# NERSC/swin_v2_weather

Measured on AMD Instinct MI355X. Metric: ERA5 samples/sec (73x721x1440) swin_73var depth12, higher is better.
Workload: dtype bf16

## Files before the change

### swin_v2_weather_amd/csrc/attn_bwd_stream.hip

```cpp
#include <stdlib.h>

#include "attn_common.h"

namespace {

typedef __attribute__((address_space(3))) unsigned lds_u32;

#ifdef SWV2_ATTNS_ARRIVE
__device__ unsigned long long attns_arr[17 * 8];
#endif

#ifdef SWV2_ATTNS_STAMPS
__device__ unsigned long long attns_stamps[512 * 8];
__device__ unsigned long long attns_win[64 * 128];
__device__ unsigned long long attns_clock[512 * 2];
#define SSTAMP_DECL unsigned long long st_prev = 0, st_acc[8] = {0, 0, 0, 0, 0, 0, 0, 0};
#define SSTAMP_START() do { asm volatile("s_memtime %0\n\ts_waitcnt lgkmcnt(0)" : "=s"(st_prev) : : "memory"); } while (0)
#define SSTAMP(k) do { unsigned long long t_; asm volatile("s_memtime %0\n\ts_waitcnt lgkmcnt(0)" : "=s"(t_) : : "memory"); \
                       st_acc[k] += t_ - st_prev; st_prev = t_; } while (0)
#else
#define SSTAMP_DECL
#define SSTAMP_START() do {} while (0)
#define SSTAMP(k) do {} while (0)
#endif
// ... 29 lines not shown
    const int lane = tid & 63;
    const int tw = __builtin_amdgcn_readfirstlane(tid >> 6);
    const int hd = blockIdx.y;
    const bool helper = tw >= PW;
    const int hw = tw - PW;

    const float tau = logit_scale[hd];
    const float sigma = __expf(fminf(tau, SWV2_LN100));
    const float sc2 = sigma * SWV2_LOG2E;
    const float inv_sc2 = 1.f / sc2;
    const int Lc = LFIX > 0 ? LFIX : L;

    if (tid < 8) ((unsigned*)(lds + OFF_CNT))[tid] = 0u;
    const unsigned lds_base = (unsigned)(uintptr_t)(lds_u32*)lds;
    const unsigned cnt_addr = lds_base + OFF_CNT;

    struct Stg { uint4 q, dO, o; float lse, rn; };
    Stg s0, s1;
    const bool two = helper && hw == HW - 1;
    auto issue = [&](int bw, int nbuf, int hidx) {
        const size_t item = (size_t)__builtin_amdgcn_readfirstlane(bw) * h + hd;
        const char* const qb = (const char*)(qkvh + item * 3 * SLAB);
        unsigned kofs = SLAB * 2, vofs = 2 * SLAB * 2;
        asm volatile("" : "+s"(kofs), "+s"(vofs));
        const char* const kb_ = qb + kofs;
        const char* const vb_ = qb + vofs;
        const char* const dob = (const char*)(doh + item * SLAB);
        const char* const ob = (const char*)(oh + item * SLAB);
        auto one = [&](Stg& st, const int craw, const unsigned lds_k) {
            const int c = min(craw, CH - 1);
            unsigned o16 = (unsigned)c * 16u, ol = (unsigned)(c / CPR) * 4u, orn = (unsigned)c * 4u;
            asm volatile("" : "+v"(o16), "+v"(ol), "+v"(orn));
            if (craw < CH) {
                asm volatile("s_mov_b32 m0, %2\n\ts_nop 0\n\tglobal_load_lds_dwordx4 %0, %1" : : "v"(o16), "s"(kb_), "s"(lds_k) : "memory");
                asm volatile("s_mov_b32 m0, %2\n\ts_nop 0\n\tglobal_load_lds_dwordx4 %0, %1" : : "v"(o16), "s"(vb_), "s"(lds_k + SLAB * 2) : "memory");
            }
            st.q = *(const uint4*)(qb + o16);
            st.dO = *(const uint4*)(dob + o16);
            st.o = *(const uint4*)(ob + o16);
            st.lse = *(const float*)((const char*)(lse + item * Lp) + ol);
            st.rn = *(const float*)((const char*)(rnorm + item * 2 * Lp) + orn);
        };
        const unsigned lds_k0 = lds_base + (unsigned)(nbuf * BUFB + B_K);
        one(s0, hidx, lds_k0 + (unsigned)hw * 1024u);
        if (two) one(s1, HT + (hidx & 63), lds_k0 + (unsigned)HT * 16u);
    };
    auto commit = [&](int buf, int hidx) {
        unsigned char* const B = lds + buf * BUFB;
        auto one = [&](const Stg& st, const int craw) {
            const int c = min(craw, CH - 1);
            const int row = c / CPR, half = c % CPR;
            float dl = 0.f;
            {
                const uint32_t a[4] = {st.dO.x, st.dO.y, st.dO.z, st.dO.w}, b[4] = {st.o.x, st.o.y, st.o.z, st.o.w};
#pragma unroll
                for (int e = 0; e < 4; ++e) {
                    dl = fmaf(__uint_as_float(a[e] << 16), __uint_as_float(b[e] << 16), dl);
                    dl = fmaf(__uint_as_float(a[e] & 0xffff0000u), __uint_as_float(b[e] & 0xffff0000u), dl);
                }
            }
            dl = group_allsum<CPR>(dl);
            uint4 aq = make_uint4(0, 0, 0, 0), ad = make_uint4(0, 0, 0, 0);
            if (half == 0) {
                const bool q_ok = row < L;
                const float lq = q_ok ? st.lse * inv_sc2 : 1.0e30f;
                uint16_t l0 = f2bf(lq);
                const float r1 = lq - bf2f(l0);
                uint16_t l1 = f2bf(r1), l2 = f2bf(r1 - bf2f(l1));
                if (!q_ok) l1 = l2 = 0;
                const uint16_t d0 = f2bf(dl);
                const float e1 = dl - bf2f(d0);
                const uint16_t d1 = f2bf(e1), d2 = f2bf(e1 - bf2f(d1));
                const uint32_t one_ = 0x3f80u, rqf = (row >= mask_thr) ? 0x3f80u : 0u;
                aq = make_uint4(l0 | ((uint32_t)l1 << 16), l2 | (one_ << 16), rqf | ((one_ - rqf) << 16), 0);
                ad = make_uint4(d0 | ((uint32_t)d1 << 16), d2, 0, 0);
            }
            if (craw < CH) {
                *(uint4*)((uint16_t*)(B + B_Q) + row * QP + half * 8) = st.q;
                *(uint4*)((uint16_t*)(B + B_DO) + row * QP + half * 8) = st.dO;
                *(uint4*)((uint16_t*)(B + B_Q) + row * QP + QSTAT + half * 8) = aq;
                *(uint4*)((uint16_t*)(B + B_DO) + row * QP + QSTAT + half * 8) = ad;
                ((float*)(B + B_RN))[c] = st.rn;
            }
        };
        one(s0, hidx);
        if (two) one(s1, HT + (hidx & 63));
    };

    int bw = blockIdx.x;
    if (bw >= Bw) return;
    if (helper) {
        issue(bw, 0, hw * 64 + lane);
        commit(0, hw * 64 + lane);
    }
    __syncthreads();

    float dsig = 0.f;
    SSTAMP_DECL
    SSTAMP_START();
#ifdef SWV2_ATTNS_STAMPS
    const unsigned long long ck0 = __builtin_amdgcn_s_memtime(), rt0 = __builtin_amdgcn_s_memrealtime();
#endif
    for (int it = 0; bw < Bw; bw += gridDim.x, ++it) {
        const int buf = it & 1;
        const size_t slab0 = ((size_t)bw * h + hd) * 3 * SLAB;
        const int bw_next = bw + gridDim.x;
        const unsigned char* const B = lds + buf * BUFB;
        const uint16_t* const Qa = (const uint16_t*)(B + B_Q);
        const uint16_t* const Da = (const uint16_t*)(B + B_DO);
        const uint16_t* const Ks = (const uint16_t*)(B + B_K);
        const uint16_t* const Vs = (const uint16_t*)(B + B_V);
        const float* const RN = (const float*)(B + B_RN);
        const unsigned target = (unsigned)(PW * (it + 1));

        int ln = lane;
        asm volatile("" : "+v"(ln));
        const int fr = ln & 15, g = ln >> 4;
        auto phase2 = [&](const int qt0, auto nq_c, auto sleep_c) {
            constexpr int NQ = decltype(nq_c)::value;
            {
                const unsigned a = cnt_addr + 4u * (unsigned)(qt0 >> 1);
                while (true) {
                    unsigned v;
                    asm volatile("ds_read_b32 %0, %1\n\ts_waitcnt lgkmcnt(0)" : "=v"(v) : "v"(a) : "memory");
                    if ((unsigned)__builtin_amdgcn_readfirstlane(v) >= target) break;
                    __builtin_amdgcn_s_sleep(decltype(sleep_c)::value);
// ... 134 lines not shown
                const f32x4 tk = mfma16(in.tq, dsb, (f32x4){0.f, 0.f, 0.f, 0.f});
                dv += tv;
                dk += tk;
                signal(NPAIR - 1);
            }
            SSTAMP(1);
            {
                const float rk = RN[Lp + key];
                float dot = 0.f;
#pragma unroll
                for (int r = 0; r < 4; ++r) dot = fmaf(dk[r], bf2f(kf[r]), dot);
                dot = xor32_allsum(xor16_allsum(dot));
                if (g == 0) dsig += dot;
                const float rks = rk * sigma;
                f32x4 v;
#pragma unroll
                for (int r = 0; r < 4; ++r) v[r] = rks * (dk[r] - bf2f(kf[r]) * dot);
                *(bf16x4*)(dqkvh + slab0 + SLAB + (size_t)key * DP + 4 * g) = f2bf4(v);
                *(bf16x4*)(dqkvh + slab0 + 2 * SLAB + (size_t)key * DP + 4 * g) = f2bf4(dv);
            }
            SSTAMP(4);
            {
                const int tt = tw == 3 ? 6 : tw == 7 ? 7 : tw == 0 ? 8 : tw == 2 ? 9 : tw == 1 ? 10 : -1;
                if (tt >= 0) {
                    SWV2_PRIO(2);
                    if (tw == 3) phase2(5, std::integral_constant<int, 1>{}, std::integral_constant<int, 1>{});
                    phase2(tt, std::integral_constant<int, 1>{}, std::integral_constant<int, 1>{});
                }
            }
        } else {
            const int hidx = hw * 64 + ln;
            if (bw_next < Bw) issue(bw_next, buf ^ 1, hidx);
            SSTAMP(0);
            if (bw_next < Bw) commit(buf ^ 1, hidx);
            SSTAMP(5);
            if (hw == 0) phase2(0, std::integral_constant<int, 2>{}, std::integral_constant<int, 4>{});
            else if (hw < HW - 1) phase2(hw + 1, std::integral_constant<int, 1>{}, std::integral_constant<int, 4>{});
        }
#ifdef SWV2_ATTNS_ARRIVE
        const bool arr_on = blockIdx.x == 3 && blockIdx.y == 0 && it >= 8 && it < 16;
        if (arr_on && lane == 0) attns_arr[tw * 8 + it - 8] = __builtin_amdgcn_s_memtime();
#endif
        __syncthreads();
#ifdef SWV2_ATTNS_ARRIVE
        if (arr_on && tid == 0) attns_arr[16 * 8 + it - 8] = __builtin_amdgcn_s_memtime();
#endif
        SSTAMP(6);
#ifdef SWV2_ATTNS_STAMPS
        if (lane == 0 && tw == 8 && blockIdx.y == 0 && blockIdx.x < 64 && it < 128) attns_win[blockIdx.x * 128 + it] = st_prev - ck0;
#endif
    }
#ifdef SWV2_ATTNS_STAMPS
    if (lane == 0 && blockIdx.y == 0 && blockIdx.x * WAVES + tw < 512) {
        for (int k = 0; k < 8; ++k) attns_stamps[(blockIdx.x * WAVES + tw) * 8 + k] = st_acc[k];
        attns_clock[(blockIdx.x * WAVES + tw) * 2] = __builtin_amdgcn_s_memtime() - ck0;
        attns_clock[(blockIdx.x * WAVES + tw) * 2 + 1] = __builtin_amdgcn_s_memrealtime() - rt0;
    }
#endif

    dsig = wave_sum(dsig);
    if (lane == 0) red[tw] = dsig;
    __syncthreads();
    if (tid == 0 && tau <= SWV2_LN100) {
        float t = 0.f;
#pragma unroll
        for (int i = 0; i < PW; ++i) t += red[i];
        atomicAdd(dlogit + hd, t * sigma);
// ... 39 lines not shown
```

### swin_v2_weather_amd/csrc/gemm.hip

```cpp
#include "common.h"

#include <cmath>
#include <cstdlib>
#include "gemm_common.h"

namespace {

constexpr int EP = 68;

struct EpiDesc {
    void* out;
    const float* bias;
    const void* aux;
    float* aux_out;
    const int32_t* rowidx;
    long ld;
    int M, N;
    int p0, p1, p2, p3, p4;
    uint32_t mg0, mg1, mg2;
    const float* loss_tar; const float* loss_qw; float* loss_part; uint16_t* loss_resid; int q0, q1, q2, q3;
};

enum { E_BF16 = 0, E_F32 = 1, E_QKV_HEADS = 2, E_GELU_GRAD = 3, E_UNPATCH = 4, E_HEADS = 5, E_F32_ACC = 6, E_BF16_GELU = 7,
       E_UNPATCH_LOSS = 8, E_UNPATCH_LOSS_SKIP = 9 };
// ... 451 lines not shown
                    const int m_g = m_w + 32 * grp;
                    const int tps = (ep.d.p1 >> 2) * (ep.d.p2 >> 2);
                    const int b0 = fdiv(min(m_g, M - 1), tps, ep.d.mg0);
                    const bool edge = (m_g + 32 >= M) || fdiv(m_g + 32, tps, ep.d.mg0) != b0;
                    float ls[8] = {0.f, 0.f, 0.f, 0.f, 0.f, 0.f, 0.f, 0.f}, ls2[8] = {0.f, 0.f, 0.f, 0.f, 0.f, 0.f, 0.f, 0.f};
#pragma unroll
                    for (int ii = 0; ii < 2; ++ii) {
                        const int i = 2 * grp + ii;
                        ep.load_tar(lrow[i], n_w + BN, ltn[i]);
                        ep.template tile_loss_t<EK == E_UNPATCH_LOSS_SKIP>(acc[i], (uint16_t*)st, lrow[i], m_w + 16 * i, n_w, lane, ls, ls2, b0, lt[i]);
                    }
                    ep.template flush<32>(ls, ls2, edge, m_g, n_w, lane);
                }
#pragma unroll
                for (int i = 0; i < RT; ++i) lt[i] = ltn[i];
                if (s + 1 < steps) commit(s + 1);
            } else {
#pragma unroll
                for (int i = 0; i < RT; ++i) {
#pragma unroll
                    for (int j = 0; j < 4; ++j)
#pragma unroll
                        for (int r = 0; r < 4; ++r) st[(4 * g + r) * EP + 16 * j + fr] = acc[i][j][r];
                    ep.tile(st, m_w + i * 16, n_w, lane);
                }
            }
        } else if constexpr (LOSS) {
            if (s + 1 < steps) commit(s + 1);
        }
    }
}

constexpr int WBM = 256, WBN = 256, WTH = 512;
__device__ __forceinline__ void dma_x4(const void* base, uint32_t byte_off, uint32_t lds_addr) {
    asm volatile("s_mov_b32 m0, %2\n\ts_nop 0\n\tglobal_load_lds_dwordx4 %0, %1" : : "v"(byte_off), "s"(base), "s"(lds_addr) : "memory");
}
template <int EK>
__device__ __forceinline__ void wide_epilogue(const Epi<EK>& ep, const f32x4 (&acc)[8][4], float* st, int m_w, int n_w, int lane) {
    const EpiDesc& d = ep.d;
    const int fr = lane & 15, g = lane >> 4;
    auto stage = [&](int i) {
#pragma unroll
        for (int j = 0; j < 4; ++j)
#pragma unroll
            for (int r = 0; r < 4; ++r) st[(4 * g + r) * EP + 16 * j + fr] = acc[i][j][r];
    };
    if constexpr (EK == E_F32 || EK == E_BF16 || EK == E_BF16_GELU || EK == E_GELU_GRAD) {
        constexpr bool F32O = EK == E_F32;
        constexpr int NQ = F32O ? 4 : 2, RQ = 16 / NQ, CW = F32O ? 4 : 8;
        const int rl = F32O ? (lane >> 4) : (lane >> 3), cl = F32O ? (lane & 15) * 4 : (lane & 7) * 8;
        const int n = n_w + cl;
        f32x4 b4[CW / 4];
#pragma unroll
        for (int q = 0; q < CW / 4; ++q) b4[q] = (f32x4){0.f, 0.f, 0.f, 0.f};
        if (d.bias) {
#pragma unroll
            for (int q = 0; q < CW / 4; ++q) b4[q] = *(const f32x4*)(d.bias + n + 4 * q);
        }
        const bool scatter = (EK == E_F32 || EK == E_BF16) && d.rowidx != nullptr;
        auto body = [&](auto scat, auto has_aux) {
            constexpr bool OPL = decltype(has_aux)::value || EK == E_GELU_GRAD;
            constexpr bool SC = decltype(scat)::value;
            [[maybe_unused]] int dstv[3][NQ];
            auto rows = [&](int i) {
                if constexpr (SC) {
#pragma unroll
                    for (int q = 0; q < NQ; ++q) dstv[i % 3][q] = d.rowidx[min(m_w + 16 * i + RQ * q + rl, d.M - 1)];
                }
            };
// ... 809 lines not shown
```

### swin_v2_weather_amd/csrc/gemm_common.h

```cpp
#pragma once
#include "common.h"

int swv2_tn_wide_launch(const swv2_operand* y, const swv2_operand* x, float* part, float* dbpart, int M, int N, int K, int S, hipStream_t st);

size_t swv2_tn_slab_ws_bytes(int C, int hidden, int heads_dp);
int swv2_tn_slab_launch(const swv2_wgrad_item* it, void* ws, size_t ws_bytes, const swv2_ln_partials* ln, hipStream_t st);

namespace {

constexpr int BM = 128, BN = 128, BK = 64;
constexpr int KCH = BK / 8;
constexpr int NTHREADS = 256;

__device__ __forceinline__ int swz(int r, int kc) { return r * BK + ((kc ^ ((r >> 1) & 7)) << 3); }

__device__ __forceinline__ void erf_parts(float x, float& erf_v, float& gauss) {
    const float z = fabsf(x) * 0.70710678118654752f;
    const float t = __builtin_amdgcn_rcpf(fmaf(0.3275911f, z, 1.f));
    gauss = __expf(-z * z);
    const float poly = t * fmaf(t, fmaf(t, fmaf(t, fmaf(t, 1.061405429f, -1.453152027f), 1.421413741f), -0.284496736f), 0.254829592f);
    const float e = fmaf(-poly, gauss, 1.f);
    erf_v = copysignf(e, x);
}
__device__ __forceinline__ int fdiv(int n, int d, uint32_t magic) {
// ... 14 lines not shown
}

constexpr int GT_LO = (127 - 14) << 7;
constexpr int GT_HALF = 18 * 128;
constexpr int GT_N = 2 * GT_HALF;
typedef unsigned short u16x2_t __attribute__((ext_vector_type(2)));

__device__ __forceinline__ uint16_t gelu_tab_arg(int i) { return (uint16_t)(((i / GT_HALF) << 15) | (GT_LO + i % GT_HALF)); }

template <int ESZ>
__device__ __forceinline__ uint32_t gelu_tab_off2(uint32_t w, bool& bad) {
    const u16x2_t a = __builtin_bit_cast(u16x2_t, w & 0x7fff7fffu);
    const u16x2_t lo = {(unsigned short)GT_LO, (unsigned short)GT_LO};
    const u16x2_t mx = {(unsigned short)(GT_HALF - 1), (unsigned short)(GT_HALF - 1)};
    const u16x2_t idx = a - lo;
    const u16x2_t idc = __builtin_elementwise_min(idx, mx);
    bad = bad || (__builtin_bit_cast(uint32_t, idx) != __builtin_bit_cast(uint32_t, idc));
    const u16x2_t sg = __builtin_bit_cast(u16x2_t, w) >> 15;
    const u16x2_t half = {(unsigned short)GT_HALF, (unsigned short)GT_HALF};
    const u16x2_t off = (idc + sg * half) * (unsigned short)ESZ;
    return __builtin_bit_cast(uint32_t, off);
}

template <int ESZ>
__device__ __forceinline__ uint32_t gelu_tab_off2_abs(uint32_t w, bool& bad) {
    const u16x2_t a = __builtin_bit_cast(u16x2_t, w & 0x7fff7fffu);
    const u16x2_t lo = {(unsigned short)GT_LO, (unsigned short)GT_LO};
    const u16x2_t mx = {(unsigned short)(GT_HALF - 1), (unsigned short)(GT_HALF - 1)};
    const u16x2_t idx = a - lo;
    const u16x2_t idc = __builtin_elementwise_min(idx, mx);
    bad = bad || (__builtin_bit_cast(uint32_t, idx) != __builtin_bit_cast(uint32_t, idc));
    const u16x2_t off = idc * (unsigned short)ESZ;
    return __builtin_bit_cast(uint32_t, off);
}

__device__ __forceinline__ uint4 pack8(const float* v) {
    uint4 r;
    r.x = f2bf2(v[0], v[1]); r.y = f2bf2(v[2], v[3]); r.z = f2bf2(v[4], v[5]); r.w = f2bf2(v[6], v[7]);
    return r;
}
__device__ __forceinline__ void unpack8(uint4 c, float* v) {
    const uint32_t w[4] = {c.x, c.y, c.z, c.w};
#pragma unroll
    for (int i = 0; i < 4; ++i) {
        v[2 * i] = __uint_as_float(w[i] << 16);
        v[2 * i + 1] = __uint_as_float(w[i] & 0xffff0000u);
    }
}

struct LoadDesc {
    const void* ptr;
    const int32_t* rowidx;
    const float* aux0;
    const float* aux1;
    const float* aux2;
    const float* aux3;
    long ld;
    int M, K;
    int p0, p1, p2, p3;
    uint32_t mg0, mg1, mg2;
};

template <int KIND> struct ALoad;

enum { A_F32 = 0, A_BF16 = 1, A_BF16_GELU = 2, A_HEADS = 3, A_PATCH = 4, A_MERGE_LN = 5, A_BF16_CS = 6 };

// ... 254 lines not shown
```

### swin_v2_weather_amd/csrc/gemm_tn.hip

```cpp
#include "gemm_common.h"

namespace {

constexpr int TM = 128;
constexpr int TP = 136;
constexpr int TCH = TM * 16 / NTHREADS;

struct TnOut {
    float* dW; float* db; const int32_t* nmap; const int32_t* kmap; int ldw, M, N, K, ntk, tiles; float* ws;
};
constexpr int TN_SMEM = 2 * TM * TP;

#ifdef SWV2_TN_STAMPS
#define TSTAMP_DECL unsigned long long st_prev = 0, st_acc[8] = {0, 0, 0, 0, 0, 0, 0, 0};
#define TSTAMP_START() do { asm volatile("s_memtime %0\n\ts_waitcnt lgkmcnt(0)" : "=s"(st_prev) : : "memory"); } while (0)
#define TSTAMP(k) do { unsigned long long t_; asm volatile("s_memtime %0\n\ts_waitcnt lgkmcnt(0)" : "=s"(t_) : : "memory"); \
                       st_acc[k] += t_ - st_prev; st_prev = t_; } while (0)
#define TSTAMP_WAITV() asm volatile("s_waitcnt vmcnt(0)" ::: "memory")
#else
#define TSTAMP_DECL
#define TSTAMP_START() do {} while (0)
#define TSTAMP(k) do {} while (0)
#define TSTAMP_WAITV() do {} while (0)
#endif
// ... 169 lines not shown
    for (int i = 0; i < 4; ++i)
#pragma unroll
        for (int j = 0; j < 4; ++j)
#pragma unroll
            for (int r = 0; r < 4; ++r) {
                int n = n_base + wr * 64 + 16 * i + 4 * g + r, k = k_base + wc * 64 + 16 * j + fr;
                if (n >= N || k >= K) continue;
                if (nmap) n = nmap[n];
                if (kmap) k = kmap[k];
                if (n >= 0 && k >= 0) atomicAdd(dW + (long)n * ldw + k, acc[i][j][r]);
            }
    if (want_db) {
#pragma unroll
        for (int e = 0; e < 8; ++e) atomicAdd(&dbs[scol * 8 + e], colsum[e]);
        __syncthreads();
        if (tid < BN && n_base + tid < N) {
            const int n = nmap ? nmap[n_base + tid] : n_base + tid;
            if (n >= 0) atomicAdd(db + n, dbs[tid]);
        }
    }
}

template <int YK, int XK, bool XG>
__global__ __launch_bounds__(NTHREADS, 2) void gemm_tn_kernel(ALoad<YK> yl, ALoad<XK> xl, TnOut o, int chunk_stride) {
    __shared__ __attribute__((aligned(16))) uint16_t smem[TN_SMEM];
    __shared__ float dbs[BN];
    __shared__ __attribute__((aligned(16))) uint16_t gtab[XK == A_BF16_GELU ? GT_N : 8];
    const int lin = blockIdx.x;
    const int x8 = lin & 7, rest = lin >> 3;
    const int tile = rest % o.tiles, slice = (rest / o.tiles) * 8 + x8;
    tn_tile<YK, XK, XG>(yl, xl, o, tile, slice, chunk_stride, smem, dbs, gtab);
}

struct TnGroup {
    ALoad<A_BF16> y0; ALoad<A_BF16_GELU> x0;
    ALoad<A_BF16> y1; ALoad<A_F32> x1;
    ALoad<A_BF16> y2; ALoad<A_HEADS> x2;
    ALoad<A_HEADS> y3; ALoad<A_F32> x3;
    TnOut o[4];
    int first[5];
    int slices;
};
__global__ __launch_bounds__(NTHREADS, 2) void gemm_tn_group_kernel(TnGroup a) {
    __shared__ __attribute__((aligned(16))) uint16_t smem[TN_SMEM];
    __shared__ float dbs[BN];
    __shared__ __attribute__((aligned(16))) uint16_t gtab[GT_N];
    const int lin = blockIdx.x, x8 = lin & 7, rest = lin >> 3, tt = a.first[4];
    const int t = rest % tt, slice = (rest / tt) * 8 + x8;
    if (t < a.first[1]) tn_tile<A_BF16, A_BF16_GELU>(a.y0, a.x0, a.o[0], t, slice, a.slices, smem, dbs, gtab);
    else if (t < a.first[2]) tn_tile<A_BF16, A_F32>(a.y1, a.x1, a.o[1], t - a.first[1], slice, a.slices, smem, dbs, gtab);
    else if (a.x2.d.p2 >= TM) {
        if (t < a.first[3]) tn_tile<A_BF16, A_HEADS, false, true>(a.y2, a.x2, a.o[2], t - a.first[2], slice, a.slices, smem, dbs, gtab);
        else tn_tile<A_HEADS, A_F32, true, true>(a.y3, a.x3, a.o[3], t - a.first[3], slice, a.slices, smem, dbs, gtab);
    } else {
        if (t < a.first[3]) tn_tile<A_BF16, A_HEADS>(a.y2, a.x2, a.o[2], t - a.first[2], slice, a.slices, smem, dbs, gtab);
        else tn_tile<A_HEADS, A_F32, true>(a.y3, a.x3, a.o[3], t - a.first[3], slice, a.slices, smem, dbs, gtab);
    }
}

struct TnReduce { TnOut o[4]; int first[5]; int slices; };
__global__ __launch_bounds__(256) void tn_reduce_kernel(TnReduce a) {
    __shared__ float part[4][64];
    const int e = blockIdx.x * 64 + (threadIdx.x & 63), sg = threadIdx.x >> 6, gt = blockIdx.y;
    const int pi = (gt >= a.first[1]) + (gt >= a.first[2]) + (gt >= a.first[3]);
    const TnOut& o = a.o[pi];
    const int tile = gt - a.first[pi], tiles = o.tiles, ntk = o.ntk;
// ... 114 lines not shown
        const TnWidePlan wp = tn_wide_plan(M, N, K);
        const int wide = getenv("SWV2_GEMM_WIDE") ? atoi(getenv("SWV2_GEMM_WIDE")) : 1;
        const bool kinds = !(YK == A_HEADS && XK == A_HEADS) && !y->rowidx && (XK == A_F32 || !x->rowidx);
        if (wide && wp.ok && kinds && ws && ws_bytes >= wp.total) {
            float* part = ws;
            float* dbpart = db ? (float*)((char*)ws + wp.part_bytes) : nullptr;
            swv2_operand xb = *x;
            if constexpr (XK == A_F32) {
                uint16_t* cb = (uint16_t*)((char*)ws + wp.part_bytes + wp.db_bytes);
                const long chunks = (long)M * (K / 8);
                hipLaunchKernelGGL(cast_rows_kernel, dim3((unsigned)((chunks + 255) / 256)), dim3(256), 0, st, (const float*)x->ptr, x->rowidx, cb,
                                   M, K, x->ld);
                xb.kind = SWV2_OP_BF16; xb.ptr = cb; xb.rowidx = nullptr; xb.ld = K;
            }
            int rc = swv2_tn_wide_launch(y, &xb, part, dbpart, M, N, K, wp.S, st);
            if (rc) return rc;
            const long quads = (long)N * K / 4;
            hipLaunchKernelGGL(tn_wide_reduce_kernel, dim3((unsigned)((quads + 255) / 256)), dim3(256), 0, st, (const float*)part,
                               (const float*)dbpart, dW, db, nmap, kmap, ldw, N, K, wp.S);
            SWV2_CHECK_LAUNCH("swv2_linear_wgrad");
            return SWV2_OK;
        }
    }
    const TnPlan p = tn_plan(M, N, K, splits);
    if (ws && ws_bytes < p.ws_bytes) {
        swv2_set_error("swv2_linear_wgrad_ws: workspace of %zu bytes, %zu needed (swv2_linear_wgrad_ws_bytes)", ws_bytes, p.ws_bytes);
        return SWV2_ERR_INVALID;
    }
    const TnOut o = tn_out(dW, db, nmap, kmap, ldw, M, N, K, ws);
    if (y->rowidx || (x->rowidx && XK != A_F32)) {
        swv2_set_error("swv2_linear_wgrad: a row gather is supported for a fp32 X operand only (dY kind %d, X kind %d)", y->kind, x->kind);
        return SWV2_ERR_UNSUPPORTED;
    }
    if constexpr (XK == A_F32) {
        if (x->rowidx)
            hipLaunchKernelGGL((gemm_tn_kernel<YK, XK, true>), dim3(p.tiles * p.slices), dim3(NTHREADS), 0, st, make_loader<YK>(y),
                               make_loader<XK>(x), o, p.real_slices);
        else
            hipLaunchKernelGGL((gemm_tn_kernel<YK, XK, false>), dim3(p.tiles * p.slices), dim3(NTHREADS), 0, st, make_loader<YK>(y),
                               make_loader<XK>(x), o, p.real_slices);
    } else {
        hipLaunchKernelGGL((gemm_tn_kernel<YK, XK, false>), dim3(p.tiles * p.slices), dim3(NTHREADS), 0, st, make_loader<YK>(y),
                           make_loader<XK>(x), o, p.real_slices);
    }
    if (ws) {
        TnReduce r = {};
        r.o[0] = o; r.first[0] = 0; r.first[1] = r.first[2] = r.first[3] = r.first[4] = p.tiles; r.slices = p.real_slices;
        hipLaunchKernelGGL(tn_reduce_kernel, dim3(BN * BN / 64, p.tiles), dim3(256), 0, st, r);
    }
    SWV2_CHECK_LAUNCH("swv2_linear_wgrad");
    return SWV2_OK;
}

template <int YK>
int launch_tn1(const swv2_operand* y, const swv2_operand* x, float* dW, float* db, const int32_t* nmap,
               const int32_t* kmap, int ldw, int M, int N, int K, int splits, float* ws, size_t wsb, hipStream_t st) {
    if (x->kind == SWV2_OP_F32) return launch_tn2<YK, A_F32>(y, x, dW, db, nmap, kmap, ldw, M, N, K, splits, ws, wsb, st);
    if constexpr (YK == A_BF16) {
        switch (x->kind) {
            case SWV2_OP_BF16: return launch_tn2<YK, A_BF16>(y, x, dW, db, nmap, kmap, ldw, M, N, K, splits, ws, wsb, st);
            case SWV2_OP_BF16_GELU: return launch_tn2<YK, A_BF16_GELU>(y, x, dW, db, nmap, kmap, ldw, M, N, K, splits, ws, wsb, st);
            case SWV2_OP_HEADS: return launch_tn2<YK, A_HEADS>(y, x, dW, db, nmap, kmap, ldw, M, N, K, splits, ws, wsb, st);
            case SWV2_OP_PATCH: return launch_tn2<YK, A_PATCH>(y, x, dW, db, nmap, kmap, ldw, M, N, K, splits, ws, wsb, st);
        }
    }
    if constexpr (YK == A_F32) {
        if (x->kind == SWV2_OP_MERGE_LN) return launch_tn2<YK, A_MERGE_LN>(y, x, dW, db, nmap, kmap, ldw, M, N, K, splits, ws, wsb, st);
// ... 109 lines not shown
```

### swin_v2_weather_amd/csrc/gemm_tn_slab.hip

```cpp
#include "gemm_common.h"
#pragma clang diagnostic ignored "-Wc++20-extensions"

namespace {

#ifdef SWV2_SLAB_PART_F32
typedef float sl_part_t;
#else
typedef uint16_t sl_part_t;
#endif
constexpr int SL_TH = 512;
constexpr int SL_SMEM = 160 * 1024;
constexpr int SL_IDX_CAP = 4096;
enum { F_ROW = 0, F_ROWG = 1, F_F32 = 2, F_F32G = 3, F_HEAD = 4 };

__device__ __forceinline__ void sl_dma(const void* base, uint32_t byte_off, uint32_t lds_addr) {
    asm volatile("s_mov_b32 m0, %2\n\ts_nop 0\n\tglobal_load_lds_dwordx4 %0, %1" : : "v"(byte_off), "s"(base), "s"(lds_addr) : "memory");
}

#ifdef SWV2_SLAB_STAMPS
#define SSTAMP_DECL unsigned long long st_prev = 0, st_acc[8] = {0, 0, 0, 0, 0, 0, 0, 0};
#define SSTAMP_START() do { asm volatile("s_memtime %0\n\ts_waitcnt lgkmcnt(0)" : "=s"(st_prev) : : "memory"); } while (0)
#define SSTAMP(k) do { unsigned long long t_; asm volatile("s_waitcnt lgkmcnt(0)\n\ts_memtime %0\n\ts_waitcnt lgkmcnt(0)" : "=s"(t_) : : "memory"); \
                       st_acc[k] += t_ - st_prev; st_prev = t_; } while (0)
#else
#define SSTAMP_DECL
#define SSTAMP_START() do {} while (0)
#define SSTAMP(k) do {} while (0)
#endif

__device__ __forceinline__ uint4 sl_gelu8_tab(uint4 w, const unsigned char* tab0, bool& bad) {
    const uint32_t in[4] = {w.x, w.y, w.z, w.w};
    uint32_t out[4], off[4];
    u16x2_t mx = {0, 0};
    const u16x2_t lo = {(unsigned short)GT_LO, (unsigned short)GT_LO};
    typedef short s16x2_t __attribute__((ext_vector_type(2)));
#pragma unroll
    for (int i = 0; i < 4; ++i) {
        const u16x2_t idx = __builtin_bit_cast(u16x2_t, in[i] & 0x7fff7fffu) - lo;
        mx = __builtin_elementwise_max(mx, idx);
        const uint32_t sg = __builtin_bit_cast(uint32_t, __builtin_bit_cast(s16x2_t, in[i]) >> 15) & (uint32_t)(GT_HALF * 0x10001u);
        off[i] = __builtin_bit_cast(uint32_t, (idx + __builtin_bit_cast(u16x2_t, sg)) << 1);
    }
#pragma unroll
    for (int i = 0; i < 4; ++i)
        out[i] = (uint32_t)*(const uint16_t*)(tab0 + (off[i] & 0xffffu)) | ((uint32_t)*(const uint16_t*)(tab0 + (off[i] >> 16)) << 16);
    const u16x2_t top = {(unsigned short)(GT_HALF - 1), (unsigned short)(GT_HALF - 1)};
    bad = __builtin_bit_cast(uint32_t, __builtin_elementwise_min(mx, top)) != __builtin_bit_cast(uint32_t, mx);
    return make_uint4(out[0], out[1], out[2], out[3]);
}

// ... 499 lines not shown
    for (int i = 0; i < 4; ++i) {
        const double xb = it[i].x.kind == SWV2_OP_F32 ? 4.0 : 2.0;
        p.ntile[i] = (N[i] / sh.TN[i]) * (K[i] / sh.TK[i]);
        cost[i] = wgt[i] * (double)it[i].dy.rows * (2.0 * N[i] * (K[i] / sh.TK[i]) + xb * K[i] * (N[i] / sh.TN[i]));
        tot += cost[i];
    }
    int used = 0;
    for (int i = 0; i < 4; ++i) {
        const int T = cdiv(it[i].dy.rows, sh.SR[i]);
        int sl = (int)(cus * cost[i] / tot / p.ntile[i] + 0.5);
        sl = std::max(1, std::min(sl, T));
        p.S[i] = sl;
        p.wgs[i] = sl * p.ntile[i];
        used += p.wgs[i];
    }
    for (int guard = 0; used != cus && guard < 64; ++guard) {
        int best = -1;
        double br = 0;
        for (int i = 0; i < 4; ++i) {
            const int T = cdiv(it[i].dy.rows, sh.SR[i]);
            if (used < cus ? (p.S[i] >= T || used + p.ntile[i] > cus) : p.S[i] <= 1) continue;
            const double r = cost[i] / p.S[i];
            if (best < 0 || (used < cus ? r > br : r < br)) { best = i; br = r; }
        }
        if (best < 0) break;
        const int d = used < cus ? 1 : -1;
        p.S[best] += d; p.wgs[best] += d * p.ntile[best]; used += d * p.ntile[best];
    }
    size_t off = 0;
    for (int i = 0; i < 4; ++i) {
        const int T = cdiv(it[i].dy.rows, sh.SR[i]);
        if ((double)it[i].dy.rows * std::max(N[i], K[i]) * 4.0 >= 4.29e9) return p;
        p.part_off[i] = off;
        off += (size_t)p.wgs[i] * sh.TN[i] * sh.TK[i] * sizeof(float);
        p.db_off[i] = off;
        off += (size_t)p.S[i] * N[i] * sizeof(float);
        off = (off + 255) / 256 * 256;
    }
    p.total = off;
    p.ok = true;
    return p;
}

SlOp sl_op(const swv2_operand& o) {
    SlOp s = {};
    s.ptr = o.ptr; s.rowidx = o.rowidx; s.ld = (int)o.ld;
    if (o.kind == SWV2_OP_HEADS) {
        s.heads = o.p[0]; s.parts = (int)o.ld; s.Lp = o.p[2]; s.DP = o.p[3];
        s.mgLp = fdiv_magic(s.Lp); s.mgDP = fdiv_magic(s.DP); s.mgH = fdiv_magic(s.heads);
    }
    return s;
}

}

size_t swv2_tn_slab_ws_bytes(int C, int hidden, int heads_dp) {
    const int set = sl_set(C, hidden, heads_dp);
    if (set < 0) return 0;
    const int cus = SL_CU_BOUND;
    const SlShape& sh = SL_SETS[set];
    size_t tile = 0;
    for (int i = 0; i < 4; ++i) tile = std::max(tile, (size_t)sh.TN[i] * sh.TK[i] * 4);
    return (size_t)cus * tile + (size_t)cus * std::max(hidden, 3 * heads_dp) * 4 + 4 * 256;
}

int swv2_tn_slab_launch(const swv2_wgrad_item* it, void* ws, size_t ws_bytes, const swv2_ln_partials* ln, hipStream_t st) {
    const int cus = sl_cus();
// ... 50 lines not shown
```

Before: 227.4.

## Add LDS-DMA weight-gradient kernel and bind m0 via asm constraint

Adds a new wgrad GEMM kernel for the column-scaled bf16×fp32 and patch-embedding operand pairs. It streams dY and X tiles straight into LDS through global_load_lds with a three-stage ring, then converts and swizzles them in place before the MFMAs, replacing register-staged loads. The LDS-DMA helpers now pass the LDS address through an {m0} constraint rather than an explicit s_mov, and the attention backward helper waits on vmcnt after its prefetch. The slab workspace partial size is also corrected to the partial element type, which shrinks the workspace when bf16 partials are used. The new path adds extra barriers and in-LDS conversion passes per stage, and it is used only when the operand shapes fit the 32-bit offset limits.

Measured after the change: 227.3 (median of 5 runs). About the same (-0.1%).

```diff
diff --git a/swin_v2_weather_amd/csrc/attn_bwd_stream.hip b/swin_v2_weather_amd/csrc/attn_bwd_stream.hip
--- a/swin_v2_weather_amd/csrc/attn_bwd_stream.hip
+++ b/swin_v2_weather_amd/csrc/attn_bwd_stream.hip
@@ -85,8 +85,8 @@
             unsigned o16 = (unsigned)c * 16u, ol = (unsigned)(c / CPR) * 4u, orn = (unsigned)c * 4u;
             asm volatile("" : "+v"(o16), "+v"(ol), "+v"(orn));
             if (craw < CH) {
-                asm volatile("s_mov_b32 m0, %2\n\ts_nop 0\n\tglobal_load_lds_dwordx4 %0, %1" : : "v"(o16), "s"(kb_), "s"(lds_k) : "memory");
-                asm volatile("s_mov_b32 m0, %2\n\ts_nop 0\n\tglobal_load_lds_dwordx4 %0, %1" : : "v"(o16), "s"(vb_), "s"(lds_k + SLAB * 2) : "memory");
+                asm volatile("s_nop 0\n\tglobal_load_lds_dwordx4 %0, %1" : : "v"(o16), "s"(kb_), "{m0}"(lds_k) : "memory");
+                asm volatile("s_nop 0\n\tglobal_load_lds_dwordx4 %0, %1" : : "v"(o16), "s"(vb_), "{m0}"(lds_k + SLAB * 2) : "memory");
             }
             st.q = *(const uint4*)(qb + o16);
             st.dO = *(const uint4*)(dob + o16);
@@ -145,6 +145,7 @@
     if (helper) {
         issue(bw, 0, hw * 64 + lane);
         commit(0, hw * 64 + lane);
+        asm volatile("s_waitcnt vmcnt(0)" ::: "memory");
     }
     __syncthreads();
 
@@ -345,7 +346,10 @@
             const int hidx = hw * 64 + ln;
             if (bw_next < Bw) issue(bw_next, buf ^ 1, hidx);
             SSTAMP(0);
-            if (bw_next < Bw) commit(buf ^ 1, hidx);
+            if (bw_next < Bw) {
+                commit(buf ^ 1, hidx);
+                asm volatile("s_waitcnt vmcnt(0)" ::: "memory");
+            }
             SSTAMP(5);
             if (hw == 0) phase2(0, std::integral_constant<int, 2>{}, std::integral_constant<int, 4>{});
             else if (hw < HW - 1) phase2(hw + 1, std::integral_constant<int, 1>{}, std::integral_constant<int, 4>{});
diff --git a/swin_v2_weather_amd/csrc/gemm.hip b/swin_v2_weather_amd/csrc/gemm.hip
--- a/swin_v2_weather_amd/csrc/gemm.hip
+++ b/swin_v2_weather_amd/csrc/gemm.hip
@@ -507,9 +507,7 @@
 }
 
 constexpr int WBM = 256, WBN = 256, WTH = 512;
-__device__ __forceinline__ void dma_x4(const void* base, uint32_t byte_off, uint32_t lds_addr) {
-    asm volatile("s_mov_b32 m0, %2\n\ts_nop 0\n\tglobal_load_lds_dwordx4 %0, %1" : : "v"(byte_off), "s"(base), "s"(lds_addr) : "memory");
-}
+__device__ __forceinline__ void dma_x4(const void* base, uint32_t byte_off, uint32_t lds_addr) { lds_dma16(base, byte_off, lds_addr); }
 template <int EK>
 __device__ __forceinline__ void wide_epilogue(const Epi<EK>& ep, const f32x4 (&acc)[8][4], float* st, int m_w, int n_w, int lane) {
     const EpiDesc& d = ep.d;
diff --git a/swin_v2_weather_amd/csrc/gemm_common.h b/swin_v2_weather_amd/csrc/gemm_common.h
--- a/swin_v2_weather_amd/csrc/gemm_common.h
+++ b/swin_v2_weather_amd/csrc/gemm_common.h
@@ -70,6 +70,10 @@
     bad = bad || (__builtin_bit_cast(uint32_t, idx) != __builtin_bit_cast(uint32_t, idc));
     const u16x2_t off = idc * (unsigned short)ESZ;
     return __builtin_bit_cast(uint32_t, off);
+}
+
+__device__ __forceinline__ void lds_dma16(const void* base, uint32_t byte_off, uint32_t lds_addr) {
+    asm volatile("s_nop 0\n\tglobal_load_lds_dwordx4 %0, %1" : : "v"(byte_off), "s"(base), "{m0}"(lds_addr) : "memory");
 }
 
 __device__ __forceinline__ uint4 pack8(const float* v) {
diff --git a/swin_v2_weather_amd/csrc/gemm_tn.hip b/swin_v2_weather_amd/csrc/gemm_tn.hip
--- a/swin_v2_weather_amd/csrc/gemm_tn.hip
+++ b/swin_v2_weather_amd/csrc/gemm_tn.hip
@@ -225,6 +225,215 @@
     tn_tile<YK, XK, XG>(yl, xl, o, tile, slice, chunk_stride, smem, dbs, gtab);
 }
 
+constexpr int DSR = 32;
+constexpr int DNS = 3;
+constexpr int DYB = DSR * BN * 2;
+constexpr int DXB = DSR * BN * 4;
+constexpr int DSTG = DYB + DXB;
+constexpr int DNIW = DSTG / 1024 / 4;
+constexpr int DCT = 32 * 8;
+static_assert(DNIW == 6 && DYB == 8 * 1024 && DXB == 16 * 1024, "stage geometry");
+
+__device__ __forceinline__ int dma_swz(int r, int c) { return r * BN + ((((c >> 4) ^ (r & 7))) << 4) + (c & 15); }
+
+template <int YK, int XK>
+__global__ __launch_bounds__(NTHREADS, 2) void gemm_tn_dma_kernel(ALoad<YK> yl, ALoad<XK> xl, TnOut o, int chunk_stride) {
+    static_assert((YK == A_BF16_CS && XK == A_F32) || (YK == A_BF16 && XK == A_PATCH), "operand pairs of the DMA path");
+    constexpr bool CS = YK == A_BF16_CS;
+    __shared__ __attribute__((aligned(1024))) unsigned char smem[DNS * DSTG];
+    __shared__ float ctab[CS ? DCT : 1];
+    const int lin = blockIdx.x;
+    const int x8 = lin & 7, rest = lin >> 3;
+    const int tile = rest % o.tiles, slice = (rest / o.tiles) * 8 + x8;
+    const int S = chunk_stride, M = o.M, N = o.N, K = o.K;
+    const int tid = threadIdx.x, lane = tid & 63, wave = __builtin_amdgcn_readfirstlane(tid >> 6);
+    const int fr = lane & 15, g = lane >> 4, wr = wave >> 1, wc = wave & 1;
+    const int tn = tile / o.ntk, tk = tile - tn * o.ntk;
+    const int n_base = tn * BN, k_base = tk * BN;
+    const int nchunks = (M + TM - 1) / TM, T32 = (M + DSR - 1) / DSR;
+    int nst = 0;
+    if (slice < S && slice < nchunks) {
+        const int nch = (nchunks - slice + S - 1) / S, last = slice + (nch - 1) * S;
+        nst = 4 * (nch - 1) + min(4, T32 - 4 * last);
+    }
+    if (nst <= 0) return;
+    auto row0_of = [&](int t) { return (slice + (t >> 2) * S) * TM + (t & 3) * DSR; };
+
+    if constexpr (CS) {
+        const int g0 = n_base >> 4, gl = (N >> 4) - 1;
+        for (int i = tid; i < DCT; i += NTHREADS) {
+            const int b = i >> 3;
+            ctab[i] = b * yl.d.p0 < M ? yl.d.aux0[b * yl.d.p2 + min(g0 + (i & 7), gl)] : 0.f;
+        }
+        __syncthreads();
+    }
+
+    int orow[DNIW];
+    uint32_t ocol[DNIW];
+#pragma unroll
+    for (int q = 0; q < DNIW; ++q) {
+        const int o16 = (wave + 4 * q) * 1024 + lane * 16;
+        if (q < 2) {
+            const int row = o16 >> 8, rem = o16 & 255, u = (rem >> 5) ^ (row & 7);
+            orow[q] = row;
+            ocol[q] = (uint32_t)min(n_base + u * 16 + ((rem >> 4) & 1) * 8, N - 8);
+        } else if constexpr (XK == A_F32) {
+            const int ox = o16 - DYB;
+            orow[q] = ox >> 9;
+            ocol[q] = (uint32_t)min(k_base + ((ox & 511) >> 2), K - 4);
+        } else {
+            const int ox = o16 - DYB, k = min(k_base + (ox >> 9) * 4, K - 4);
+            orow[q] = (ox & 511) >> 4;
+            ocol[q] = (uint32_t)(((k >> 4) * xl.d.p1 + ((k >> 2) & 3)) * xl.d.p2);
+        }
+    }
+    const uint32_t lds0 = (uint32_t)(uintptr_t)smem + (uint32_t)(wave * 1024);
+    auto issue = [&](int t, int slot) {
+        const int r0 = row0_of(t);
+        const uint32_t ls = lds0 + (uint32_t)(slot * DSTG);
+#pragma unroll
+        for (int q = 0; q < DNIW; ++q) {
+            const int m = min(r0 + orow[q], M - 1);
+            uint32_t off;
+            if (q < 2) off = 2u * ((uint32_t)m * (uint32_t)yl.d.ld + ocol[q]);
+            else if constexpr (XK == A_F32) off = 4u * ((uint32_t)m * (uint32_t)xl.d.ld + ocol[q]);
+            else {
+                const int W = xl.d.p2, gw = W >> 2, gh = xl.d.p1 >> 2, Ct = xl.d.p3 ? xl.d.p3 : xl.d.p0;
+                const int b = fdiv(m, gh * gw, xl.d.mg0), ij = m - b * gh * gw, i = fdiv(ij, gw, xl.d.mg1), j = ij - i * gw;
+                off = 4u * ((uint32_t)b * (uint32_t)(Ct * xl.d.p1 * W) + ocol[q] + (uint32_t)(4 * i * W + 4 * j));
+            }
+            lds_dma16(q < 2 ? yl.d.ptr : xl.d.ptr, off, ls + (uint32_t)(q * 4 * 1024));
+        }
+    };
+
+    f32x4 acc[4][4], accdb[4];
+#pragma unroll
+    for (int i = 0; i < 4; ++i) {
+        accdb[i] = (f32x4){0.f, 0.f, 0.f, 0.f};
+#pragma unroll
+        for (int j = 0; j < 4; ++j) acc[i][j] = (f32x4){0.f, 0.f, 0.f, 0.f};
+    }
+    const bool want_db = o.db != nullptr && tk == 0;
+    const bool db_wave = want_db && wc == 0;
+    const bf16x8 ones = {0x3F80, 0x3F80, 0x3F80, 0x3F80, 0x3F80, 0x3F80, 0x3F80, 0x3F80};
+
+    issue(0, 0);
+    if (nst > 1) issue(1, 1);
+    for (int t = 0; t < nst; ++t) {
+        if (t + 1 < nst) asm volatile("s_waitcnt vmcnt(%0)" : : "n"(DNIW) : "memory");
+        else asm volatile("s_waitcnt vmcnt(0)" ::: "memory");
+        __builtin_amdgcn_sched_barrier(0);
+        __builtin_amdgcn_s_barrier();
+        __builtin_amdgcn_sched_barrier(0);
+        if (t + 2 < nst) issue(t + 2, (t + 2) % DNS);
+        unsigned char* const sb = smem + (t % DNS) * DSTG;
+        const int r0 = row0_of(t);
+        uint4 cx[2];
+#pragma unroll
+        for (int p = 0; p < 2; ++p) {
+            const int c = tid + NTHREADS * p;
+            int row;
+            RawF32 v;
+            if constexpr (XK == A_F32) {
+                row = c >> 4;
+                const float* src = (const float*)(sb + DYB) + row * BN + (c & 15) * 8;
+                v = {*(const f32x4*)src, *(const f32x4*)(src + 4)};
+            } else {
+                row = c & 31;
+                const float* src = (const float*)(sb + DYB) + ((c >> 5) * 2 * DSR + row) * 4;
+                v = {*(const f32x4*)src, *(const f32x4*)(src + DSR * 4)};
+            }
+            cx[p] = r0 + row < M ? cvt_f32x8(v) : make_uint4(0, 0, 0, 0);
+            const int yrow = c >> 4;
+            uint4* const yp = (uint4*)(sb + c * 16);
+            if constexpr (CS) {
+                const int m = r0 + yrow, u = ((c & 15) >> 1) ^ (yrow & 7);
+                const int gi = (min(n_base + u * 16, N - 16) >> 4) - (n_base >> 4);
+                const RawCS rv = {*yp, m < M ? ctab[fdiv(m, yl.d.p0, yl.d.mg0) * 8 + gi] : 0.f};
+                *yp = m < M ? yl.cvt(rv) : make_uint4(0, 0, 0, 0);
+            } else {
+                if (r0 + DSR > M && r0 + yrow >= M) *yp = make_uint4(0, 0, 0, 0);
+            }
+        }
+        __syncthreads();
+#pragma unroll
+        for (int p = 0; p < 2; ++p) {
+            const int c = tid + NTHREADS * p;
+            const int row = XK == A_F32 ? c >> 4 : c & 31, ch = XK == A_F32 ? c & 15 : c >> 5;
+            *(uint4*)((uint16_t*)(sb + DYB) + dma_swz(row, ch * 8)) = cx[p];
+        }
+        __syncthreads();
+        const uint16_t* const Ys = (const uint16_t*)sb;
+        const uint16_t* const Xs = (const uint16_t*)(sb + DYB);
+        const int ra = 8 * g + (fr >> 2), cc = (fr & 3) * 4;
+        bf16x8 af[4], bf[4];
+#pragma unroll
+        for (int i = 0; i < 4; ++i) {
+            const bf16x4 a0 = lds_tr_read(Ys + dma_swz(ra, wr * 64 + i * 16) + cc);
+            const bf16x4 a1 = lds_tr_read(Ys + dma_swz(ra + 4, wr * 64 + i * 16) + cc);
+            const bf16x4 b0 = lds_tr_read(Xs + dma_swz(ra, wc * 64 + i * 16) + cc);
+            const bf16x4 b1 = lds_tr_read(Xs + dma_swz(ra + 4, wc * 64 + i * 16) + cc);
+            af[i] = __builtin_shufflevector(a0, a1, 0, 1, 2, 3, 4, 5, 6, 7);
+            bf[i] = __builtin_shufflevector(b0, b1, 0, 1, 2, 3, 4, 5, 6, 7);
+        }
+#pragma unroll
+        for (int i = 0; i < 4; ++i)
+#pragma unroll
+            for (int j = 0; j < 4; ++j) acc[i][j] = mfma32(af[i], bf[j], acc[i][j]);
+        if (db_wave) {
+#pragma unroll
+            for (int i = 0; i < 4; ++i) accdb[i] = mfma32(af[i], ones, accdb[i]);
+        }
+    }
+    asm volatile("s_waitcnt vmcnt(0)" ::: "memory");
+    if (o.ws) {
+        float* pt = o.ws + ((size_t)slice * o.tiles + tile) * (BN * BN);
+#pragma unroll
+        for (int i = 0; i < 4; ++i)
+#pragma unroll
+            for (int j = 0; j < 4; ++j)
+#pragma unroll
+                for (int r = 0; r < 4; ++r)
+                    pt[(wr * 64 + 16 * i + 4 * g + r) * BN + wc * 64 + 16 * j + fr] = acc[i][j][r];
+    } else {
+#pragma unroll
+        for (int i = 0; i < 4; ++i)
+#pragma unroll
+            for (int j = 0; j < 4; ++j)
+#pragma unroll
+                for (int r = 0; r < 4; ++r) {
+                    int n = n_base + wr * 64 + 16 * i + 4 * g + r, k = k_base + wc * 64 + 16 * j + fr;
+                    if (n >= N || k >= K) continue;
+                    if (o.nmap) n = o.nmap[n];
+                    if (o.kmap) k = o.kmap[k];
+                    if (n >= 0 && k >= 0) atomicAdd(o.dW + (long)n * o.ldw + k, acc[i][j][r]);
+                }
+    }
+    if (db_wave && fr == 0) {
+#pragma unroll
+        for (int i = 0; i < 4; ++i)
+#pragma unroll
+            for (int r = 0; r < 4; ++r) {
+                int n = n_base + wr * 64 + 16 * i + 4 * g + r;
+                if (n >= N) continue;
+                if (o.nmap) n = o.nmap[n];
+                if (n >= 0) atomicAdd(o.db + n, accdb[i][r]);
+            }
+    }
+}
+
+template <int YK, int XK>
+bool tn_dma_covers(const swv2_operand* y, const swv2_operand* x, int M) {
+    if (y->rowidx || x->rowidx || (double)M * (double)y->ld * 2.0 >= 4.29e9) return false;
+    if constexpr (YK == A_BF16_CS && XK == A_F32) return (double)M * (double)x->ld * 4.0 < 4.29e9 && cdiv(M, y->p[0]) <= DCT / 8;
+    if constexpr (YK == A_BF16 && XK == A_PATCH) {
+        const int Cin = x->p[0], H = x->p[1], W = x->p[2], Ct = x->p[3] ? x->p[3] : Cin;
+        const double samples = (double)cdiv(M, (H / 4) * (W / 4));
+        return !x->aux0 && samples * Ct * H * W * 4.0 < 4.29e9;
+    }
+    return false;
+}
+
 struct TnGroup {
     ALoad<A_BF16> y0; ALoad<A_BF16_GELU> x0;
     ALoad<A_BF16> y1; ALoad<A_F32> x1;
@@ -405,7 +614,15 @@
         swv2_set_error("swv2_linear_wgrad: a row gather is supported for a fp32 X operand only (dY kind %d, X kind %d)", y->kind, x->kind);
         return SWV2_ERR_UNSUPPORTED;
     }
-    if constexpr (XK == A_F32) {
+    bool dma = false;
+    if constexpr ((YK == A_BF16_CS && XK == A_F32) || (YK == A_BF16 && XK == A_PATCH)) {
+        dma = tn_dma_covers<YK, XK>(y, x, M);
+        if (dma)
+            hipLaunchKernelGGL((gemm_tn_dma_kernel<YK, XK>), dim3(p.tiles * p.slices), dim3(NTHREADS), 0, st, make_loader<YK>(y),
+                               make_loader<XK>(x), o, p.real_slices);
+    }
+    if (dma) {
+    } else if constexpr (XK == A_F32) {
         if (x->rowidx)
             hipLaunchKernelGGL((gemm_tn_kernel<YK, XK, true>), dim3(p.tiles * p.slices), dim3(NTHREADS), 0, st, make_loader<YK>(y),
                                make_loader<XK>(x), o, p.real_slices);
diff --git a/swin_v2_weather_amd/csrc/gemm_tn_slab.hip b/swin_v2_weather_amd/csrc/gemm_tn_slab.hip
--- a/swin_v2_weather_amd/csrc/gemm_tn_slab.hip
+++ b/swin_v2_weather_amd/csrc/gemm_tn_slab.hip
@@ -13,9 +13,7 @@
 constexpr int SL_IDX_CAP = 4096;
 enum { F_ROW = 0, F_ROWG = 1, F_F32 = 2, F_F32G = 3, F_HEAD = 4 };
 
-__device__ __forceinline__ void sl_dma(const void* base, uint32_t byte_off, uint32_t lds_addr) {
-    asm volatile("s_mov_b32 m0, %2\n\ts_nop 0\n\tglobal_load_lds_dwordx4 %0, %1" : : "v"(byte_off), "s"(base), "s"(lds_addr) : "memory");
-}
+__device__ __forceinline__ void sl_dma(const void* base, uint32_t byte_off, uint32_t lds_addr) { lds_dma16(base, byte_off, lds_addr); }
 
 #ifdef SWV2_SLAB_STAMPS
 #define SSTAMP_DECL unsigned long long st_prev = 0, st_acc[8] = {0, 0, 0, 0, 0, 0, 0, 0};
@@ -581,7 +579,8 @@
         const int T = cdiv(it[i].dy.rows, sh.SR[i]);
         if ((double)it[i].dy.rows * std::max(N[i], K[i]) * 4.0 >= 4.29e9) return p;
         p.part_off[i] = off;
-        off += (size_t)p.wgs[i] * sh.TN[i] * sh.TK[i] * sizeof(float);
+        off += (size_t)p.wgs[i] * sh.TN[i] * sh.TK[i] * sizeof(sl_part_t);
+        off = (off + 15) / 16 * 16;
         p.db_off[i] = off;
         off += (size_t)p.S[i] * N[i] * sizeof(float);
         off = (off + 255) / 256 * 256;
```
